# olsonanl/close_kmers

Measured on AMD Instinct MI355X. Metric: protein residues/s vs 1B-entry kmer image; 1/2/4/8 MI355X, higher is better.
Workload: dtype u64

## Files before the change

### close_kmers_amd/csrc/kgx_host_batch.cpp

```cpp
#include <hip/hip_runtime.h>

#include <algorithm>
#include <chrono>
#include <cstdio>
#include <cstdlib>
#include <cstring>
#include <string>
#include <vector>

#include "kgx_rt.h"

using namespace kgx;

extern "C" {


namespace {

void cut_at_nul(char *b, uint64_t len)
{
    const void *z = len ? std::memchr(b, 0, len) : nullptr;
    if (z) {
        const uint64_t slen = (uint64_t)((const char *)z - b);
        for (uint64_t i = slen ? slen - 1 : 0; i < len; i++)
// ... 870 lines not shown
    return KGX_OK;
}

hipError_t own_queue_stream(int device, hipStream_t *s)
{
    (void)device;
    const char *e = std::getenv("KGX_OWN_QUEUES");
    if (!e || std::atoi(e) != 0) {
        int least = 0, greatest = 0;
        if (hipDeviceGetStreamPriorityRange(&least, &greatest) == hipSuccess && least != greatest &&
            hipStreamCreateWithPriority(s, hipStreamNonBlocking, least) == hipSuccess)
            return hipSuccess;
        (void)hipGetLastError();
    }
    return hipStreamCreateWithFlags(s, hipStreamNonBlocking);
}

int process_batch_chunked(kgx_ctx *c, const kgx_params *params, const char *residues,
                          const uint64_t *seq_offsets, uint32_t n_seq, uint32_t want, uint32_t K,
                          kgx_result *out)
{
    if (!c->twin) {
        int rc = kgx_ctx_create(c->img, &c->twin);
        if (rc)
            return rc;
    }
    kgx_ctx *t = c->twin;
    t->opt.probe_variant = c->opt.probe_variant;
    t->opt.probe_j = c->opt.probe_j;
    t->opt.probe_filter = c->opt.probe_filter;
    t->opt.probe_serialize = c->opt.probe_serialize;
    t->opt.score_variant = c->opt.score_variant;
    t->opt.score_wave_tiles = c->opt.score_wave_tiles;
    kgx_ctx *xs[2] = {c, t};
    if (!c->copy_stream)
        HIP_TRY(own_queue_stream(c->img->device, &c->copy_stream));
    if (c->opt.host_upload_stream && !c->up_stream)
        HIP_TRY(own_queue_stream(c->img->device, &c->up_stream));
    for (auto *ev : {&c->chunk_counts, &c->chunk_gathered, &c->chunk_done, &c->chunk_h2d})
        if (int erc = ensure_events(*ev, K))
            return erc;

    const uint64_t r0 = seq_offsets[0], n_res = seq_offsets[n_seq] - r0;
    std::vector<uint32_t> cut(K + 1, 0);
    cut[K] = n_seq;
    const bool taper = c->opt.host_taper && K >= 3;
    const double wsum = taper ? (double)K - 1.0 : (double)K;
    for (uint32_t k = 1; k < K; k++) {
        const double before = taper ? 0.5 + (double)(k - 1) : (double)k;
        const uint64_t target = r0 + (uint64_t)((double)n_res * before / wsum);
        uint32_t s = (uint32_t)(std::lower_bound(seq_offsets, seq_offsets + n_seq + 1, target) - seq_offsets);
        cut[k] = std::min(std::max(s, cut[k - 1]), n_seq);
    }
    cut.erase(std::unique(cut.begin(), cut.end()), cut.end());
    K = (uint32_t)cut.size() - 1;
    const bool want_calls = (want & KGX_WANT_CALLS) != 0;
    const bool want_otu = (want & KGX_WANT_OTU) != 0;
    const bool need_hits = (want & KGX_WANT_HITS) != 0;
    const bool want_best = (want & KGX_WANT_BEST) != 0;
    uint64_t hbase = 0, cbase = 0, obase = 0, nwin = 0;
    const bool compact = c->opt.host_hits16 && need_hits && c->img->layout == KGX_LAYOUT_PACKED16;
    uint64_t mbase = 0;
    int rc = reset_chunked_results(c, n_seq, want_best, compact);
    if (rc)
        return rc;
    struct PoolDrain {
// ... 652 lines not shown
```

### close_kmers_amd/csrc/kgx_internal.h

```cpp
#ifndef KGX_INTERNAL_H
#define KGX_INTERNAL_H

#include <hip/hip_runtime.h>
#include <stdint.h>

#include "kgx.h"
#include "kgx_line_home.h"

namespace kgx {

constexpr int KMER = 8;
constexpr uint64_t CORE = 1280000000ULL;
constexpr uint64_t MAX_ENCODED = 25600000000ULL;
constexpr uint64_t EMPTY_KEY = MAX_ENCODED + 1;
constexpr int RUN_CAP = 40000 - 2;

constexpr int PROBE_WAVES = 4;
constexpr uint32_t HIT_PLANES = KGX_HIT_PLANES, HIT_PACKED16 = KGX_HIT_PACKED16;
constexpr int PROBE_BUCKET = 0;
constexpr int PROBE_KEY_FIRST = 1;
constexpr int PROBE_AUTO = -1;
constexpr int PROBE_LINE = 2;
constexpr int PROBE_LINE8 = 3;
constexpr int PROBE_J_DEFAULT = 2;
// ... 94 lines not shown
    uint32_t n_seq;
    uint64_t max_tiles;
};
struct ProbeHits {
    uint4 *hot, *cold;
    uint64_t *hit_mask;
};
struct ProbeRun {
    int probe_j;
    int variant;
    uint32_t lds_kb;
    uint32_t max_blocks;
    bool defer;
    uint32_t nt;
};
hipError_t launch_probe(const ProbeBatch &b, const ProbeTable &t, const ProbeHits &h, const ProbeRun &r,
                        hipStream_t stream);
hipError_t launch_probe_dna(const ProbeBatch &b, const ProbeTable &t, const ProbeHits &h, const ProbeRun &r,
                            hipStream_t stream);

hipError_t launch_pack(const kgx_sig_kmer *table, packed_bucket *packed, uint64_t n,
                       uint32_t *not_packable, hipStream_t stream);
hipError_t launch_unpack(const packed_bucket *packed, kgx_sig_kmer *out, uint64_t n,
                         hipStream_t stream);
hipError_t launch_filter_build(const void *table, int layout, uint64_t num_sigs, uint64_t *filter,
                               uint32_t log2_words, hipStream_t stream);

enum { SCORE_HYBRID = 0, SCORE_WAVE = 1, SCORE_LANE = 2, SCORE_WAVE_ONLY = 3  };
constexpr uint32_t LONG_SEQ = 2048;
hipError_t launch_score(uint32_t n_seq, uint64_t n_residues, const uint64_t *wbase, const uint32_t *tile_seq,
                        uint64_t max_tiles, const uint64_t *hit_mask, uint32_t tile_windows, uint4 *hot,
                        kgx_call *calls, void *ranges, uint32_t *hit_count, uint32_t *call_count,
                        kgx_params params, uint32_t want, uint32_t hit_format, int variant, uint32_t wave_tiles,
                        const uint32_t *plan_status, hipStream_t stream);
hipError_t launch_best_calls(uint32_t n_seq, const kgx_call *calls, const uint64_t *start, const uint32_t *count,
                             kgx_call *ws, kgx_best_call *out, hipStream_t stream);
hipError_t launch_otus(uint32_t n_seq, const uint64_t *wbase, const uint64_t *hit_mask, uint32_t tile_windows,
                       const uint4 *hot, const uint4 *cold, int32_t *ws, kgx_otu *otus, uint32_t *otu_count,
                       uint32_t hit_format, hipStream_t stream);

constexpr uint32_t SMALL_GATHER_SEQ = 256;
constexpr uint32_t SMALL_COLLECT_BEST_SEQ = 8192;
constexpr uint32_t SMALL_GATHER_BLOCKS = 64;
hipError_t launch_small_gather(uint32_t n, const uint64_t *wbase, const uint64_t *hit_mask, uint32_t tile_windows,
                               const uint32_t *hit_count, const uint32_t *call_count, const uint4 *hot,
                               const uint4 *cold, const kgx_call *calls, const uint32_t *otu_count,
                               const kgx_otu *otus, kgx_hit *hits_out, kgx_call *calls_out, kgx_otu *otus_out,
                               uint64_t *h0, uint64_t *h1, uint64_t *h2, const uint32_t *status,
                               const kgx_best_call *best, kgx_best_call *best_host, uint32_t *status_host,
                               uint64_t *nwin_host, uint32_t *done_host, uint32_t token, uint32_t *blocks_done,
                               uint32_t hit_format, hipStream_t stream);
hipError_t launch_gather(uint32_t n_seq, const uint64_t *wbase, const uint64_t *hit_mask,
                         uint32_t tile_windows, const uint32_t *call_count, const uint4 *hot, const uint4 *cold,
                         const kgx_call *calls, const uint64_t *hit_dense_off,
                         const uint64_t *call_dense_off, kgx_hit *hits_out, kgx_call *calls_out,
                         uint32_t seq_base, uint32_t hit_format, const uint32_t *otu_count, const kgx_otu *otus,
                         const uint64_t *otu_dense_off, kgx_otu *otus_out, hipStream_t stream,
                         uint4 *hits16_out = nullptr,
                         uint32_t *hits12_out = nullptr);
size_t count_scan_workspace_bytes(uint32_t n);
hipError_t launch_count_scan(uint32_t n, const uint32_t *c0, const uint32_t *c1, const uint32_t *c2, uint64_t *o0,
                             uint64_t *o1, uint64_t *o2, void *workspace, hipStream_t stream);
constexpr int SMALL_PIECES = 5;
struct SmallPieces {
    uint4 *dst[SMALL_PIECES];
    const uint4 *src[SMALL_PIECES];
    uint64_t end16[SMALL_PIECES];
// ... 99 lines not shown
```

### close_kmers_amd/csrc/kgx_options.h

```cpp
#pragma once

#include <cstdint>
#include <cstring>
#include <string>

namespace kgx {

inline bool probe_j_supported(int j) { return (j >= 1 && j <= 5) || j == 8; }

struct CtxOptions {
    int64_t probe_variant = -1;
    int64_t probe_j = 2;
    int64_t probe_lds_kb = 0;
    int64_t probe_persist = 0;
    int64_t probe_filter = 1;
    int64_t line_index = 1;
    int64_t probe_nt = 0;
    int64_t probe_serialize = 1;
    int64_t probe_stream = 0;
    int64_t plan_fused = 0;
    int64_t score_variant = 0;
    int64_t score_wave_tiles = 16;
    int64_t fq_residues = 1;
    int64_t fq_count = 1;
    int64_t fq_probe_j = 1;
    int64_t fq_plan = 1;
    int64_t fq_fused = 1;
    int64_t microbench_span = 0;
    int64_t microbench_ilp = 8;
    int64_t microbench_wgs = 8;
    int64_t host_chunks = 6;
    int64_t host_copy = 1;
    int64_t host_copy_blocks = 64;
    int64_t host_hits16 = 1;
    int64_t host_threads = 12;
    int64_t stage_threads = 8;
    int64_t host_upload_stream = 0;
    int64_t host_score_variant = 1;
    int64_t host_stream = 1;
    int64_t host_taper = 1;
    int64_t pinned_input = 1;
    int64_t host_rec12 = 1;
    int64_t host_h2d_first = 1;
    int64_t host_stage_all = 0;
    int64_t host_stream_dma = 0;
    int64_t host_nt = 1;
    int64_t counts_first = 1;
    int64_t host_profile = 0;
    int64_t small_batch = 1 << 21;
    int64_t small_wave = 1;
    int64_t small_wave_tiles = 1;
    int64_t small_fused = 0;
    int64_t fused_inline = 1;
    int64_t gunzip_device = 0;
};
// ... 26 lines not shown
    {KGX_OPT(stage_threads), 1, 64, "1..64", nullptr},
    {KGX_OPT(host_score_variant), -1, 2, "-1 (the context's score_variant) or 0..2", nullptr},
    {KGX_OPT(host_upload_stream), 0, 1, "0 or 1", nullptr},
    {KGX_OPT(host_stream_dma), 0, 1, "0 or 1", nullptr},
    {KGX_OPT(pinned_input), 0, 1, "0 or 1", nullptr},
    {KGX_OPT(host_stage_all), 0, 1, "0 or 1", nullptr},
    {KGX_OPT(host_h2d_first), 0, 1, "0 or 1", nullptr},
    {KGX_OPT(host_rec12), 0, 1, "0 or 1", nullptr},
    {KGX_OPT(host_nt), 0, 1, "0 or 1", nullptr},
    {KGX_OPT(host_taper), 0, 1, "0 or 1", nullptr},
    {KGX_OPT(host_stream), 0, 1, "0 or 1", nullptr},
    {KGX_OPT(counts_first), 0, 1, "0 or 1", nullptr},
    {KGX_OPT(host_threads), 1, 64, "1..64", nullptr},
    {KGX_OPT(small_batch), 0, 1 << 24, "0..16777216 residues", nullptr},
    {KGX_OPT(probe_stream), 0, 1, "0 or 1", nullptr},
    {KGX_OPT(probe_persist), 0, 32, "0..32 workgroups per CU", nullptr},
    {KGX_OPT(small_wave), 0, 1, "0 or 1", nullptr},
    {KGX_OPT(host_profile), 0, 1, "0 or 1", nullptr},
    {KGX_OPT(host_chunks), 1, 64, "1..64", nullptr},
    {KGX_OPT(fq_count), 0, 1, "0 or 1", nullptr},
    {KGX_OPT(fq_residues), 0, 1, "0 or 1", nullptr},
    {KGX_OPT(score_variant), 0, 2, "0, 1 or 2", nullptr},
    {KGX_OPT(probe_lds_kb), 0, 160, "0..160", nullptr},
    {KGX_OPT(fused_inline), 0, 1, "0 or 1", nullptr},
    {KGX_OPT(small_fused), 0, 1, "0 or 1", nullptr},
    {KGX_OPT(small_wave_tiles), 1, 256, "1..256", nullptr},
    {KGX_OPT(score_wave_tiles), 1, 256, "1..256", nullptr},
    {KGX_OPT(fq_fused), 0, 1, "0 or 1", nullptr},
    {KGX_OPT(fq_plan), 0, 1, "0 or 1", nullptr},
    {KGX_OPT(fq_probe_j), 0, 4, "0 (= probe_j), 1, 2, 3 or 4", nullptr},
    {KGX_OPT(probe_j), 0, 0, "1, 2, 3, 4, 5 or 8", probe_j_ok},
};
constexpr size_t CTX_OPTION_COUNT = sizeof(CTX_OPTION_TABLE) / sizeof(CTX_OPTION_TABLE[0]);
static const CtxOptionRow CTX_OPTION_TABLE_IO[] = {
    {KGX_OPT(gunzip_device), 0, 1, "0 or 1", nullptr},
};
#undef KGX_OPT

inline const CtxOptionRow *ctx_option_find(const char *name)
{
    for (const CtxOptionRow &r : CTX_OPTION_TABLE)
        if (!std::strcmp(r.name, name))
            return &r;
    for (const CtxOptionRow &r : CTX_OPTION_TABLE_IO)
        if (!std::strcmp(r.name, name))
            return &r;
    return nullptr;
}

inline int ctx_option_set(CtxOptions &o, const char *name, int64_t value, std::string *err)
{
    const CtxOptionRow *r = ctx_option_find(name);
    if (!r) {
        *err = std::string("unknown option ") + name;
        return -1;
    }
    if (r->ok ? !r->ok(value) : (value < r->lo || value > r->hi)) {
        *err = std::string(name) + " must be " + r->must_be;
        return -1;
    }
    o.*(r->field) = value;
    return 0;
}

inline bool ctx_option_get(const CtxOptions &o, const char *name, int64_t *value)
{
    const CtxOptionRow *r = ctx_option_find(name);
    if (r)
        *value = o.*(r->field);
    return r != nullptr;
}

}
```

### close_kmers_amd/csrc/kgx_rt.h

```cpp
#ifndef KGX_RT_H
#define KGX_RT_H

#include <hip/hip_runtime.h>

#include <algorithm>
#include <atomic>
#include <chrono>
#include <condition_variable>
#include <cstdio>
#include <cstdlib>
#include <cstring>
#include <deque>
#include <functional>
#include <memory>
#include <mutex>
#include <string>
#include <thread>
#include <vector>

#include "kgx_internal.h"
#include "kgx_options.h"

namespace kgx {

// ... 373 lines not shown
        fqc_calls;
    kgx::PinnedVec<uint32_t> h_fqc_n, h_fqc_reads, h_fqc_fc, h_fqc_len;
    kgx::PinnedVec<uint64_t> h_fqc_tot, h_fqc_fo, h_fqc_coff;
    kgx::PinnedVec<kgx_call> h_fqc_calls;
    kgx::CtxOptions opt;
    bool probe_defer = true;
    std::vector<uint64_t> h_hoff, h_coff, h_ooff;
    kgx::PinnedVec<kgx_hit> h_hits;
    kgx::PinnedVec<kgx_call> h_calls;
    kgx::PinnedVec<kgx_otu> h_otus;
    kgx::PinnedVec<uint32_t> h_ocount;
    kgx::DevBuf otu_ws, otus, otu_count, dense_ooff, dense_otus;
    bool have_otus = false;
    kgx::PinnedVec<uint32_t> h_hcount, h_ccount;
    kgx::PinnedVec<char> h_res;
    kgx_ctx *twin = nullptr;
    kgx::PinnedVec<uint64_t> h_off_stage, h_dense_hoff, h_dense_coff, h_dense_ooff, h_nwin;
    std::unique_ptr<kgx::HostPool> pool;
    std::unique_ptr<kgx::HostPool> stage_pool;
    kgx::PinnedVec<uint4> h_hits16;
    kgx::PinnedVec<uint64_t> h_mask;
    std::vector<uint64_t> h_wstart;
    std::vector<hipEvent_t> chunk_done;
    std::vector<hipEvent_t> chunk_counts;
    std::vector<hipEvent_t> chunk_gathered;
    hipStream_t copy_stream = nullptr;
    hipStream_t up_stream = nullptr;
    kgx::DevBuf up_res, up_off;
    kgx::DevBuf dense_mask, dense_best;
    double rate_hits = 0.35, rate_calls = 0.05, rate_otus = 0.05;
    uint64_t stream_fallbacks = 0;
    bool one_pass_pinned = false;
    uint64_t pinned_batches = 0, nul_reruns = 0;
    uint32_t counts_enqueued = 0;
    kgx::PinnedVec<uint32_t> h_nul;
    std::vector<hipEvent_t> chunk_h2d;
    kgx::DevBuf dense_counts, cscan_ws;
    kgx::PinnedVec<uint32_t> h_counts;
    kgx::PinnedVec<uint32_t> h_hits12;
    kgx::PinnedVec<char> h_res_all;
    kgx::PinnedVec<uint64_t> h_off_all;
    kgx::PinnedVec<uint4> h_small;
    kgx::PinnedVec<uint32_t> h_done;
    kgx::DevBuf small_blocks_done;
    uint64_t fused_batches = 0, small_batches = 0;
    kgx::PinnedVec<uint64_t> h_fwb;
    kgx::PinnedVec<kgx_hit> h_fhits;
    kgx::PinnedVec<kgx_call> h_fcalls;
    kgx::PinnedVec<uint32_t> h_fcounts, h_fdone;
    kgx::PinnedVec<uint64_t> h_fdbg;
    uint32_t small_token = 0;
    kgx::PinnedVec<kgx_call> h_calls_region;
    kgx::PinnedVec<kgx_otu> h_otus_region;
    int compact_out = 0;
    struct CompactSeg {
        uint32_t s0, s1, words;
        uint64_t hit_begin, rec_at, mask_at;
    };
    std::vector<CompactSeg> compact_segs;
    std::vector<kgx_hit_chunk> compact_chunks;
    std::vector<hipEvent_t> prof_ev;
    std::vector<hipEvent_t> prof_done;
    kgx_host_profile last_profile{};
    std::unique_ptr<kgx::RollupScratch> rollup;
};

// ... 55 lines not shown
```

### close_kmers_amd/csrc/kgx_runtime.cpp

```cpp
#include <hip/hip_runtime.h>
#include <sched.h>

#include <algorithm>
#include <cerrno>
#include <ctime>
#include <chrono>
#include <cstdio>
#include <cstdlib>
#include <cstring>
#include <map>
#include <stdexcept>
#include <string>
#include <atomic>
#include <fcntl.h>
#include <mutex>
#include <sys/stat.h>
#include <thread>
#include <unistd.h>
#include <vector>

#include "kgx_rt.h"

using namespace kgx;

// ... 831 lines not shown
    bool ok = std::fwrite(&h, sizeof(h), 1, f) == 1;
    const uint64_t chunk = 1ull << 25;
    std::vector<kgx_sig_kmer> buf(std::min(chunk, std::max<uint64_t>(img->num_sigs, 1)));
    for (uint64_t b = 0; ok && b < img->num_sigs; b += chunk) {
        const uint64_t m = std::min(chunk, img->num_sigs - b);
        int rc = image_read(img, b, m, buf.data());
        if (rc) {
            std::fclose(f);
            return rc;
        }
        ok = std::fwrite(buf.data(), sizeof(kgx_sig_kmer), m, f) == m;
    }
    if (std::fclose(f) != 0)
        ok = false;
    return ok ? KGX_OK : fail(KGX_EIO, "short write to " + path);
}


int kgx_ctx_create(kgx_image *img, kgx_ctx **out)
{
    if (!img || !out)
        return fail(KGX_EINVAL, "null argument");
    HIP_TRY(hipSetDevice(img->device));
    bool probe_defer = true;
    if (int rc = env_switch("KGX_PROBE_DEFER", "rounds per slice", "deferred", probe_defer))
        return rc;
    int64_t gunzip_device = CtxOptions{}.gunzip_device;
    if (const char *g = std::getenv("KGX_GUNZIP_DEVICE")) {
        if (*g && std::strcmp(g, "0") && std::strcmp(g, "1"))
            return fail(KGX_EINVAL, std::string("KGX_GUNZIP_DEVICE: 0 (host threads) or 1 (device), not \"") + g + "\"");
        if (*g)
            gunzip_device = *g == '1';
    }
    kgx_ctx *c = new kgx_ctx;
    c->img = img;
    c->probe_defer = probe_defer;
    c->opt.gunzip_device = gunzip_device;
    hipError_t e = hipStreamCreateWithFlags(&c->stream, hipStreamNonBlocking);
    if (e != hipSuccess) {
        delete c;
        return fail(KGX_EDEVICE, std::string("stream: ") + hipGetErrorString(e));
    }
    c->own_stream = true;
    if (const char *sb = std::getenv("KGX_SMALL_BATCH"))
        c->opt.small_batch = std::min<int64_t>(1 << 24, std::max<int64_t>(0, std::atoll(sb)));
    e = hipEventCreateWithFlags(&c->probe_done, hipEventDisableTiming);
    if (e != hipSuccess) {
        (void)hipStreamDestroy(c->stream);
        delete c;
        return fail(KGX_EDEVICE, std::string("event: ") + hipGetErrorString(e));
    }
    *out = c;
    return KGX_OK;
}

int kgx_ctx_destroy(kgx_ctx *c)
{
    if (!c)
        return KGX_OK;
    (void)hipSetDevice(c->img->device);
    if (c->twin)
        kgx_ctx_destroy(c->twin);
    (void)hipStreamSynchronize(c->stream);
    for (DevBuf *b : {&c->residues, &c->offsets, &c->wbase, &c->tile_seq, &c->hit_mask,
                      &c->hits, &c->calls, &c->hit_count, &c->call_count, &c->dense_hoff,
                      &c->dense_coff, &c->dense_hits, &c->dense_calls, &c->plan_ws, &c->ranges})
        b->release();
    {
        std::lock_guard<std::mutex> lock(c->img->probe_mu);
        if (c->img->last_probe == c->probe_done)
// ... 246 lines not shown
    return probe_chained(c, [&] {
        const CtxProbe p = ctx_probe(c, bases, n_bases, anchors);
        return launch_probe_dna(p.batch, ctx_probe_table(c), p.hits, p.run, c->stream);
    });
}

}

extern "C" {

int kgx_stage_probe(kgx_ctx *c, const uint8_t *d_res, const uint64_t *d_off)
{
    if (!c || (!d_res && c->n_residues) || d_off != c->d_off)
        return fail(KGX_EINVAL, "probe: residues missing or offsets differ from the plan");
    return probe_chained(c, [&] {
        const CtxProbe p = ctx_probe(c, d_res, c->n_residues, d_off);
        return launch_probe(p.batch, ctx_probe_table(c), p.hits, p.run, c->stream);
    });
}



int kgx_stage_score(kgx_ctx *c, const kgx_params *params, uint32_t want)
{
    if (!c)
        return fail(KGX_EINVAL, "null ctx");
    kgx_params p;
    if (params)
        p = *params;
    else
        kgx_params_default(&p);
    HIP_TRY(hipSetDevice(c->img->device));
    const bool best = (want & KGX_WANT_BEST) != 0;
    HIP_TRY(launch_score(c->n_seq, c->n_residues, c->wbase.as<uint64_t>(), c->tile_seq.as<uint32_t>(), c->max_tiles,
                         c->hit_mask.as<uint64_t>(), c->tile_windows, c->hits.as<uint4>(), c->calls.as<kgx_call>(),
                         c->ranges.p, c->hit_count.as<uint32_t>(), c->call_count.as<uint32_t>(), p,
                         want | (best ? KGX_WANT_CALLS : 0u), c->hit_format, c->opt.score_variant,
                         (uint32_t)c->opt.score_wave_tiles, c->plan_status.as<uint32_t>(), c->stream));
    c->have_best = false;
    c->have_otus = false;
    if (want & KGX_WANT_OTU) {
        HIP_TRY(c->otu_ws.reserve(std::max<uint64_t>(c->hit_slots, 1) * sizeof(int32_t)));
        HIP_TRY(c->otus.reserve(std::max<uint64_t>(c->hit_slots, 1) * sizeof(kgx_otu)));
        HIP_TRY(c->otu_count.reserve(std::max<uint64_t>(c->n_seq, 1) * sizeof(uint32_t)));
        HIP_TRY(launch_otus(c->n_seq, c->wbase.as<uint64_t>(), c->hit_mask.as<uint64_t>(), c->tile_windows,
                            c->hits.as<uint4>(), c->hits.as<uint4>() + c->hit_slots, c->otu_ws.as<int32_t>(),
                            c->otus.as<kgx_otu>(), c->otu_count.as<uint32_t>(), c->hit_format, c->stream));
        c->have_otus = true;
    }
    if (best) {
        HIP_TRY(c->best.reserve(std::max<uint64_t>(c->n_seq, 1) * sizeof(kgx_best_call)));
        HIP_TRY(c->best_ws.reserve(c->hit_slots * sizeof(kgx_call)));
        if (!c->defer_best)
            HIP_TRY(launch_best_calls(c->n_seq, c->calls.as<kgx_call>(), c->wbase.as<uint64_t>(),
                                      c->call_count.as<uint32_t>(), c->best_ws.as<kgx_call>(),
                                      c->best.as<kgx_best_call>(), c->stream));
        c->have_best = true;
    }
    return KGX_OK;
}

int kgx_find_best_calls(kgx_ctx *c, const kgx_call *calls, const uint64_t *call_offsets, uint32_t n_seq,
                        kgx_best_call *out)
{
    if (!c || (n_seq && (!call_offsets || !out)))
        return fail(KGX_EINVAL, "null argument");
    if (n_seq == 0)
        return KGX_OK;
    const uint64_t c0 = call_offsets[0], n = call_offsets[n_seq] - c0;
    if (n && !calls)
        return fail(KGX_EINVAL, "null calls");
// ... 90 lines not shown
                               c->tile_windows, c->plan_status.as<uint32_t>(), c->plan_ws.as<uint32_t>(), c->stream);
        if (e != hipSuccess)
            rc = fail(KGX_EDEVICE, std::string("fq plan: ") + hipGetErrorString(e));
    }
    if (!rc)
        rc = stage_probe_dna(c, fr->bases, fr->n_bases, fr->anchors, fr->offsets);
    c->opt.probe_j = keep_j;
    if (rc)
        return rc;
    if ((rc = kgx_stage_score(c, params, want)))
        return rc;
    return out ? kgx_device_result_get(c, out) : KGX_OK;
}

}

extern "C" {

int kgx_ctx_stat(kgx_ctx *c, const char *name, int64_t *value)
{
    if (!c || !name || !value)
        return fail(KGX_EINVAL, "null argument");
    const std::string n = name;
    if (n == "fused_batches")
        *value = (int64_t)c->fused_batches;
    else if (n == "small_batches")
        *value = (int64_t)c->small_batches;
    else if (n == "stream_fallbacks")
        *value = (int64_t)c->stream_fallbacks;
    else if (n == "pinned_batches")
        *value = (int64_t)c->pinned_batches;
    else if (n == "nul_reruns")
        *value = (int64_t)c->nul_reruns;
    else
        return fail(KGX_EINVAL, "unknown statistic " + n);
    return KGX_OK;
}

int kgx_ctx_host_profile(kgx_ctx *c, kgx_host_profile *out)
{
    if (!c || !out)
        return fail(KGX_EINVAL, "null argument");
    *out = c->last_profile;
    return KGX_OK;
}

int kgx_device_batch_collect(kgx_ctx *c, uint32_t want, kgx_result *out)
{
    if (!c || !out)
        return fail(KGX_EINVAL, "null argument");
    if (!c->have_hits)
        return fail(KGX_EINVAL, "no device batch to collect");
    const bool want_calls = (want & KGX_WANT_CALLS) != 0;
    const bool want_otu = (want & KGX_WANT_OTU) != 0;
    const bool need_hits = (want & KGX_WANT_HITS) != 0;
    const bool want_best = (want & KGX_WANT_BEST) != 0;
    if (want_otu && !c->have_otus)
        return fail(KGX_EINVAL, "no device OTU tallies (score with KGX_WANT_OTU)");
    if (want_best && !c->have_best)
        return fail(KGX_EINVAL, "no device best calls (score with KGX_WANT_BEST)");
    HIP_TRY(hipSetDevice(c->img->device));
    PhaseTimer tm(c);
    const uint32_t n_seq = c->n_seq;
    const bool best_now = want_best && n_seq && !need_hits && !want_calls && !want_otu;
    if (c->counts_enqueued != want + 1) {
        if (int rc = kgx::collect_counts_enqueue(c, want))
// ... 233 lines not shown
```

### close_kmers_amd/csrc/kgx_score.hip

```cpp
#include "kgx_device.h"
#include "kgx_lstd.h"

namespace kgx {


template <class F>
__device__ __forceinline__ uint32_t for_each_run(const uint64_t *__restrict__ hit_mask,
                                                 uint32_t tile_windows, uint64_t gw0, uint64_t gw1,
                                                 F &&f)
{
    if (gw0 >= gw1)
        return 0;
    const uint32_t J = tile_windows / 64;
    const uint64_t gfirst = gw0 >> 6, glast = (gw1 - 1) >> 6;
    uint64_t tile = gfirst / J;
    uint32_t pre = 0;
    for (uint64_t g = tile * J; g < gfirst; g++)
        pre += (uint32_t)__popcll(hit_mask[g]);
    uint32_t ordinal = 0;
    uint64_t next = hit_mask[gfirst];
    for (uint64_t g = gfirst; g <= glast; g++) {
        if (g != gfirst && g % J == 0) {
            tile = g / J;
            pre = 0;
        }
        const uint64_t full = next;
        if (g < glast)
            next = hit_mask[g + 1];
        const uint32_t lo = g == gfirst ? (uint32_t)(gw0 & 63) : 0u;
        const uint32_t hi = g == glast ? (uint32_t)((gw1 - 1) & 63) + 1 : 64u;
        const uint64_t bits = full & bit_range(lo, hi);
        const uint32_t cnt = (uint32_t)__popcll(bits);
        if (cnt)
            f(tile * tile_windows + pre + (uint32_t)__popcll(full & bit_range(0, lo)), cnt, ordinal, bits,
              (uint32_t)(64 * g - gw0));
        ordinal += cnt;
        pre += (uint32_t)__popcll(full);
    }
    return ordinal;
}


struct RunTail {
    uint32_t pos, fI, idx;
    float wt;
    uint32_t avg;
    uint32_t fb;
    uint64_t at;
};

constexpr int SCORE_BATCH = 8;

template <bool PK, int SB = SCORE_BATCH>
__device__ __forceinline__ void score_sequence(
    uint32_t s, const uint64_t *__restrict__ wbase, const uint64_t *__restrict__ hit_mask,
    uint32_t tile_windows, uint4 *__restrict__ hot, kgx_call *__restrict__ calls,
    uint2 *__restrict__ ranges, uint32_t *__restrict__ hit_count, uint32_t *__restrict__ call_count,
    const kgx_params &prm, uint32_t want)
{
    const uint64_t gw0 = wbase[s], gw1 = wbase[s + 1];
    const bool want_calls = (want & KGX_WANT_CALLS) != 0;
    const bool want_otu = (want & KGX_WANT_OTU) != 0;
    if (!want_calls && !want_otu) {
        hit_count[s] = for_each_run(hit_mask, tile_windows, gw0, gw1,
                                    [](uint64_t, uint32_t, uint32_t, uint64_t, uint32_t) {});
        call_count[s] = 0;
        return;
    }
    if (!want_otu && prm.min_hits > 0 && gw1 > gw0) {
        uint32_t nh = 0;
        for (uint64_t g = gw0 >> 6; g <= (gw1 - 1) >> 6; g++) {
            const uint32_t lo = g == (gw0 >> 6) ? (uint32_t)(gw0 & 63) : 0u;
            const uint32_t hi = g == ((gw1 - 1) >> 6) ? (uint32_t)((gw1 - 1) & 63) + 1 : 64u;
            nh += (uint32_t)__popcll(hit_mask[g] & bit_range(lo, hi));
        }
        if ((int)nh < prm.min_hits) {
            hit_count[s] = nh;
            call_count[s] = 0;
            return;
        }
    }

    typedef HitFields<PK> HF;
    constexpr uint32_t F_RUN = KGX_HIT_IN_RUN << HF::FLAG_SHIFT, F_CNT = KGX_HIT_COUNTED << HF::FLAG_SHIFT,
                       F_OTU = KGX_HIT_OTU << HF::FLAG_SHIFT;
    constexpr int FD = HF::FLAG_DWORD;
    uint32_t *hw = reinterpret_cast<uint32_t *>(hot);
    const uint64_t cbase = gw0;
    const uint32_t gap = (uint32_t)prm.max_gap;
    int n = 0;
    uint32_t cur = 0, first_pos = 0, last_pos = 0, last_idx = 0, run_start = 0;
    int cnt = 0;
    float wsum = 0.0f;
    RunTail p1 = {0, 0, 0, 0.0f, 0, 0, 0}, p2 = {0, 0, 0, 0.0f, 0, 0, 0};
    uint32_t ncalls = 0;

    auto flush = [&]() {
        if (n == 0)
            return;
        if (cnt >= prm.min_hits && wsum >= (float)prm.min_weighted_hits) {
            if (want_calls) {
                kgx_call cl;
                cl.start = first_pos;
                cl.end = last_pos + (KMER - 1);
                cl.count = cnt;
                cl.function_index = cur;
                cl.weighted_hits = wsum;
                calls[cbase + ncalls] = cl;
            }
            if (want_otu)
                ranges[cbase + ncalls] = make_uint2(run_start, last_idx);
            ncalls++;
        }
        if (n >= 2 && p2.fI != cur && p2.fI == p1.fI) {
            cur = p1.fI;
            n = 2;
            run_start = p2.idx;
            first_pos = p2.pos;
            cnt = 2;
            wsum = 0.0f + p2.wt;
            wsum = wsum + p1.wt;
            last_pos = p1.pos;
            last_idx = p1.idx;
            if (want_otu) {
                hw[4 * p2.at + FD] = p2.fb | F_RUN | F_CNT;
                hw[4 * p1.at + FD] = p1.fb | F_RUN | F_CNT;
            }
        } else {
            n = 0;
        }
    };

    auto step = [&](const uint4 &r, uint32_t i, uint64_t at, uint32_t pos) {
        const uint32_t avg = HF::avg(r);
        const uint32_t fI = HF::fi(r);
        const float wt = __uint_as_float(HF::wt(r));
        const uint32_t fb = HF::flag_base(r);
        if (n > 0 && p1.pos + gap < pos) {
            if (n >= prm.min_hits)
                flush();
            else
                n = 0;
        }
        if (n == 0) {
            cur = fI;
            cnt = 0;
            wsum = 0.0f;
            run_start = i;
            first_pos = pos;
        }
        bool accept = true;
        if (prm.order_constraint && n > 0) {
            const uint32_t d = (pos - p1.pos) - (uint32_t)((int)p1.avg - (int)avg);
            accept = (fI == p1.fI) && d <= 20u;
        }
        if (accept) {
            if (n < RUN_CAP) {
                n++;
                const bool counted = fI == cur;
                if (want_otu)
                    hw[4 * at + FD] = fb | F_RUN | (counted ? F_CNT : 0u);
                if (counted) {
                    cnt++;
                    wsum += wt;
                    last_pos = pos;
                    last_idx = i;
                }
                p2 = p1;
                p1 = RunTail{pos, fI, i, wt, avg, fb, at};
            }
            if (n > 1 && cur != fI && p2.fI == p1.fI)
                flush();
        }
    };

    auto load_batch = [&](uint4 *rb, uint64_t at0, uint32_t b, uint32_t c) {
#pragma unroll
        for (int k = 0; k < SB; k++)
            if (b + k < c)
                rb[k] = hot[at0 + b + k];
    };
    const uint32_t nh = for_each_run(hit_mask, tile_windows, gw0, gw1,
                                     [&](uint64_t at0, uint32_t c, uint32_t ord0, uint64_t bits, uint32_t pbase) {
        uint4 ra[SB], rb[SB];
        load_batch(ra, at0, 0, c);
        for (uint32_t b = 0; b < c; b += 2 * SB) {
            if (b + SB < c)
                load_batch(rb, at0, b + SB, c);
#pragma unroll
            for (int k = 0; k < SB; k++)
                if (b + k < c) {
                    step(ra[k], ord0 + b + k, at0 + b + k, pbase + (uint32_t)__builtin_ctzll(bits));
                    bits &= bits - 1;
                }
            if (b + SB >= c)
                break;
            if (b + 2 * SB < c)
                load_batch(ra, at0, b + 2 * SB, c);
#pragma unroll
            for (int k = 0; k < SB; k++)
                if (b + SB + k < c) {
                    step(rb[k], ord0 + b + SB + k, at0 + b + SB + k,
                         pbase + (uint32_t)__builtin_ctzll(bits));
                    bits &= bits - 1;
                }
        }
    });
    if (n >= prm.min_hits)
        flush();
    hit_count[s] = nh;
    call_count[s] = want_calls ? ncalls : 0;

    if (want_otu && ncalls > 0) {
        uint32_t ci = 0;
        uint2 rg = ranges[cbase];
        const uint32_t end = ranges[cbase + ncalls - 1].y;
        for_each_run(hit_mask, tile_windows, gw0, gw1,
                     [&](uint64_t at0, uint32_t c, uint32_t ord0, uint64_t, uint32_t) {
            for (uint32_t k = 0; k < c; k++) {
                const uint32_t i = ord0 + k;
                if (i > end)
                    return;
                while (i > rg.y)
                    rg = ranges[cbase + ++ci];
                if (i >= rg.x) {
                    const uint32_t f = hw[4 * (at0 + k) + FD];
                    if (f & F_CNT)
                        hw[4 * (at0 + k) + FD] = f | F_OTU;
                }
            }
        });
    }
}

template <bool PK, int SB>
__global__ __launch_bounds__(256) void score_kernel(
    uint32_t n_seq, const uint64_t *__restrict__ wbase, const uint64_t *__restrict__ hit_mask,
    uint32_t tile_windows, uint4 *__restrict__ hot, kgx_call *__restrict__ calls,
    uint2 *__restrict__ ranges, uint32_t *__restrict__ hit_count, uint32_t *__restrict__ call_count,
    kgx_params prm, uint32_t want, uint32_t skip_above)
{
    for (uint32_t s = blockIdx.x * blockDim.x + threadIdx.x; s < n_seq; s += gridDim.x * blockDim.x) {
        const uint64_t w = wbase[s + 1] - wbase[s];
        if (w > skip_above && w <= (uint64_t)RUN_CAP)
            continue;
        score_sequence<PK, SB>(s, wbase, hit_mask, tile_windows, hot, calls, ranges, hit_count, call_count, prm,
                               want);
    }
}


constexpr uint32_t SQ = 256;

struct ScoreQueue {
    uint32_t pos[SQ];
    uint32_t seq[SQ];
    uint32_t at[SQ];
    uint64_t mw[64];
    uint64_t wb[65];
};


__device__ __forceinline__ uint32_t seq_lower_bound(const uint64_t *__restrict__ wbase,
                                                    const uint32_t *__restrict__ tile_seq, uint32_t T, uint64_t x)
{
    uint32_t s = tile_seq[x / T];
    if (wbase[s] < x)
        return s + 1;
    while (s > 0 && wbase[s - 1] == x)
        s--;
    return s;
}

template <bool PK>
__global__ __launch_bounds__(256) void score_wave_kernel(
    uint32_t n_seq, const uint64_t *__restrict__ wbase, const uint32_t *__restrict__ tile_seq,
    const uint64_t *__restrict__ hit_mask, uint32_t tile_windows, uint32_t wave_tiles, uint4 *__restrict__ hot,
    kgx_call *__restrict__ calls, uint32_t *__restrict__ hit_count, uint32_t *__restrict__ call_count,
    kgx_params prm, uint32_t want, uint32_t only_above, const uint32_t *__restrict__ plan_status)
{
// ... 299 lines not shown
    }
    flush_counts(s_hi);
    if (!scoring)
        return;
    if (qtail != qissue)
        issue(qtail - qissue);
    if (npend) {
        wave_lds_sync();
        process_chunk(npend, rpend);
    }
    if (o_valid) {
        close_open();
        if (lane == 0)
            call_count[o_seq] = want_calls ? o_ncalls : 0u;
    }
}

template <bool PK>
__global__ __launch_bounds__(256) void score_long_kernel(
    uint32_t n_seq, const uint64_t *__restrict__ wbase, const uint64_t *__restrict__ hit_mask,
    uint32_t tile_windows, uint4 *__restrict__ hot, kgx_call *__restrict__ calls,
    uint2 *__restrict__ ranges, uint32_t *__restrict__ hit_count, uint32_t *__restrict__ call_count,
    kgx_params prm, uint32_t want)
{
    const uint32_t s = blockIdx.x * blockDim.x + threadIdx.x;
    if (s < n_seq && wbase[s + 1] - wbase[s] > (uint64_t)RUN_CAP)
        score_sequence<PK>(s, wbase, hit_mask, tile_windows, hot, calls, ranges, hit_count, call_count, prm, want);
}

hipError_t launch_score(uint32_t n_seq, uint64_t n_residues, const uint64_t *wbase, const uint32_t *tile_seq,
                        uint64_t max_tiles, const uint64_t *hit_mask, uint32_t tile_windows, uint4 *hot,
                        kgx_call *calls, void *ranges, uint32_t *hit_count, uint32_t *call_count,
                        kgx_params params, uint32_t want, uint32_t hit_format, int variant, uint32_t wave_tiles,
                        const uint32_t *plan_status, hipStream_t stream)
{
    if (n_seq == 0)
        return hipSuccess;
    const bool pk = hit_format == HIT_PACKED16;
    const dim3 lanes((n_seq + 255) / 256);
    const bool wave_ok = !params.order_constraint && max_tiles * tile_windows < (1ull << 32);
    wave_tiles = std::max<uint32_t>(1, wave_tiles);
    const uint64_t waves = std::max<uint64_t>(1, (max_tiles + wave_tiles - 1) / wave_tiles);
    const dim3 wgrid((uint32_t)((waves + 3) / 4));
#define KGX_WAVE(P, ABOVE)                                                                                      \
    hipLaunchKernelGGL(score_wave_kernel<P>, wgrid, dim3(256), 0, stream, n_seq, wbase, tile_seq, hit_mask,     \
                       tile_windows, wave_tiles, hot, calls, hit_count, call_count, params, want, (ABOVE), plan_status)
    if (variant == SCORE_WAVE_ONLY && wave_ok) {
        if (pk)
            KGX_WAVE(true, 0u);
        else
            KGX_WAVE(false, 0u);
        return hipGetLastError();
    }
    if ((variant == SCORE_WAVE || variant == SCORE_WAVE_ONLY) && wave_ok) {
        if (pk) {
            KGX_WAVE(true, 0u);
            hipLaunchKernelGGL(score_long_kernel<true>, lanes, dim3(256), 0, stream, n_seq, wbase, hit_mask,
                               tile_windows, hot, calls, static_cast<uint2 *>(ranges), hit_count, call_count, params,
                               want);
        } else {
            KGX_WAVE(false, 0u);
            hipLaunchKernelGGL(score_long_kernel<false>, lanes, dim3(256), 0, stream, n_seq, wbase, hit_mask,
                               tile_windows, hot, calls, static_cast<uint2 *>(ranges), hit_count, call_count, params,
                               want);
        }
        return hipGetLastError();
    }
    const bool hybrid = variant == SCORE_HYBRID && wave_ok;
    const uint32_t skip = hybrid ? LONG_SEQ : ~0u;
    const bool small = n_residues < 64ull * n_seq;
    static const uint32_t grid_cap = [] {
        const char *e = std::getenv("KGX_SCORE_GRID_CAP");
        return e ? (uint32_t)std::max(0L, std::strtol(e, nullptr, 10)) : 0u;
    }();
    const dim3 sgrid(grid_cap ? std::min<uint32_t>(lanes.x, grid_cap) : lanes.x);
#define KGX_SCORE(P, B)                                                                                          \
    hipLaunchKernelGGL((score_kernel<P, B>), sgrid, dim3(256), 0, stream, n_seq, wbase, hit_mask, tile_windows, hot, \
                       calls, static_cast<uint2 *>(ranges), hit_count, call_count, params, want, skip)
    if (pk && small)
        KGX_SCORE(true, 2);
    else if (pk)
        KGX_SCORE(true, SCORE_BATCH);
    else if (small)
        KGX_SCORE(false, 2);
    else
        KGX_SCORE(false, SCORE_BATCH);
#undef KGX_SCORE
    if (hybrid) {
        if (pk)
            KGX_WAVE(true, LONG_SEQ);
        else
            KGX_WAVE(false, LONG_SEQ);
    }
#undef KGX_WAVE
    return hipGetLastError();
}

__global__ __launch_bounds__(256) void best_call_kernel(uint32_t n_seq, const kgx_call *__restrict__ calls,
                                                        const uint64_t *__restrict__ start,
                                                        const uint32_t *__restrict__ count, kgx_call *__restrict__ ws,
                                                        kgx_best_call *__restrict__ out)
{
    const uint32_t s = blockIdx.x * blockDim.x + threadIdx.x;
    if (s < n_seq)
        out[s] = best_call_decide(calls + start[s], count[s], ws + start[s]);
}

hipError_t launch_best_calls(uint32_t n_seq, const kgx_call *calls, const uint64_t *start, const uint32_t *count,
                             kgx_call *ws, kgx_best_call *out, hipStream_t stream)
{
    if (n_seq == 0)
        return hipSuccess;
    hipLaunchKernelGGL(best_call_kernel, dim3((n_seq + 255) / 256), dim3(256), 0, stream, n_seq, calls, start,
                       count, ws, out);
    return hipGetLastError();
}


constexpr int64_t OTU_LDS = 24;
// ... 80 lines not shown
```

Before: 64.74 billion.

## Add lean lane scorer with 32-bit indices, narrow hit loads, optional wave compaction

Result: faster. 66.79 billion, median of 6 (+3.2%).

```diff
diff --git a/close_kmers_amd/csrc/kgx_host_batch.cpp b/close_kmers_amd/csrc/kgx_host_batch.cpp
--- a/close_kmers_amd/csrc/kgx_host_batch.cpp
+++ b/close_kmers_amd/csrc/kgx_host_batch.cpp
@@ -926,6 +926,7 @@
     t->opt.probe_serialize = c->opt.probe_serialize;
     t->opt.score_variant = c->opt.score_variant;
     t->opt.score_wave_tiles = c->opt.score_wave_tiles;
+    t->opt.score_lean = c->opt.score_lean;
     kgx_ctx *xs[2] = {c, t};
     if (!c->copy_stream)
         HIP_TRY(own_queue_stream(c->img->device, &c->copy_stream));
diff --git a/close_kmers_amd/csrc/kgx_internal.h b/close_kmers_amd/csrc/kgx_internal.h
--- a/close_kmers_amd/csrc/kgx_internal.h
+++ b/close_kmers_amd/csrc/kgx_internal.h
@@ -150,7 +150,7 @@
                         uint64_t max_tiles, const uint64_t *hit_mask, uint32_t tile_windows, uint4 *hot,
                         kgx_call *calls, void *ranges, uint32_t *hit_count, uint32_t *call_count,
                         kgx_params params, uint32_t want, uint32_t hit_format, int variant, uint32_t wave_tiles,
-                        const uint32_t *plan_status, hipStream_t stream);
+                        int lean, const uint32_t *plan_status, hipStream_t stream, bool *lean_taken = nullptr);
 hipError_t launch_best_calls(uint32_t n_seq, const kgx_call *calls, const uint64_t *start, const uint32_t *count,
                              kgx_call *ws, kgx_best_call *out, hipStream_t stream);
 hipError_t launch_otus(uint32_t n_seq, const uint64_t *wbase, const uint64_t *hit_mask, uint32_t tile_windows,
diff --git a/close_kmers_amd/csrc/kgx_options.h b/close_kmers_amd/csrc/kgx_options.h
--- a/close_kmers_amd/csrc/kgx_options.h
+++ b/close_kmers_amd/csrc/kgx_options.h
@@ -21,6 +21,7 @@
     int64_t plan_fused = 0;
     int64_t score_variant = 0;
     int64_t score_wave_tiles = 16;
+    int64_t score_lean = 1;
     int64_t fq_residues = 1;
     int64_t fq_count = 1;
     int64_t fq_probe_j = 1;
@@ -113,8 +114,9 @@
     {KGX_OPT(probe_j), 0, 0, "1, 2, 3, 4, 5 or 8", probe_j_ok},
 };
 constexpr size_t CTX_OPTION_COUNT = sizeof(CTX_OPTION_TABLE) / sizeof(CTX_OPTION_TABLE[0]);
-static const CtxOptionRow CTX_OPTION_TABLE_IO[] = {
+static const CtxOptionRow CTX_OPTION_TABLE_LATER[] = {
     {KGX_OPT(gunzip_device), 0, 1, "0 or 1", nullptr},
+    {KGX_OPT(score_lean), 0, 2, "0, 1 or 2", nullptr},
 };
 #undef KGX_OPT
 
@@ -123,7 +125,7 @@
     for (const CtxOptionRow &r : CTX_OPTION_TABLE)
         if (!std::strcmp(r.name, name))
             return &r;
-    for (const CtxOptionRow &r : CTX_OPTION_TABLE_IO)
+    for (const CtxOptionRow &r : CTX_OPTION_TABLE_LATER)
         if (!std::strcmp(r.name, name))
             return &r;
     return nullptr;
diff --git a/close_kmers_amd/csrc/kgx_rt.h b/close_kmers_amd/csrc/kgx_rt.h
--- a/close_kmers_amd/csrc/kgx_rt.h
+++ b/close_kmers_amd/csrc/kgx_rt.h
@@ -429,6 +429,7 @@
     uint64_t stream_fallbacks = 0;
     bool one_pass_pinned = false;
     uint64_t pinned_batches = 0, nul_reruns = 0;
+    uint64_t lean_scores = 0;
     uint32_t counts_enqueued = 0;
     kgx::PinnedVec<uint32_t> h_nul;
     std::vector<hipEvent_t> chunk_h2d;
diff --git a/close_kmers_amd/csrc/kgx_runtime.cpp b/close_kmers_amd/csrc/kgx_runtime.cpp
--- a/close_kmers_amd/csrc/kgx_runtime.cpp
+++ b/close_kmers_amd/csrc/kgx_runtime.cpp
@@ -887,10 +887,19 @@
         if (*g)
             gunzip_device = *g == '1';
     }
+    int64_t score_lean = CtxOptions{}.score_lean;
+    if (const char *l = std::getenv("KGX_SCORE_LEAN")) {
+        if (*l && std::strcmp(l, "0") && std::strcmp(l, "1") && std::strcmp(l, "2"))
+            return fail(KGX_EINVAL, std::string("KGX_SCORE_LEAN: 0 (general lane scorer), 1 (lean) or 2 (lean, "
+                                                "packed), not \"") + l + "\"");
+        if (*l)
+            score_lean = *l - '0';
+    }
     kgx_ctx *c = new kgx_ctx;
     c->img = img;
     c->probe_defer = probe_defer;
     c->opt.gunzip_device = gunzip_device;
+    c->opt.score_lean = score_lean;
     hipError_t e = hipStreamCreateWithFlags(&c->stream, hipStreamNonBlocking);
     if (e != hipSuccess) {
         delete c;
@@ -1203,11 +1212,14 @@
         kgx_params_default(&p);
     HIP_TRY(hipSetDevice(c->img->device));
     const bool best = (want & KGX_WANT_BEST) != 0;
+    bool lean_taken = false;
     HIP_TRY(launch_score(c->n_seq, c->n_residues, c->wbase.as<uint64_t>(), c->tile_seq.as<uint32_t>(), c->max_tiles,
                          c->hit_mask.as<uint64_t>(), c->tile_windows, c->hits.as<uint4>(), c->calls.as<kgx_call>(),
                          c->ranges.p, c->hit_count.as<uint32_t>(), c->call_count.as<uint32_t>(), p,
                          want | (best ? KGX_WANT_CALLS : 0u), c->hit_format, c->opt.score_variant,
-                         (uint32_t)c->opt.score_wave_tiles, c->plan_status.as<uint32_t>(), c->stream));
+                         (uint32_t)c->opt.score_wave_tiles, (int)c->opt.score_lean, c->plan_status.as<uint32_t>(),
+                         c->stream, &lean_taken));
+    c->lean_scores += lean_taken;
     c->have_best = false;
     c->have_otus = false;
     if (want & KGX_WANT_OTU) {
@@ -1364,6 +1376,8 @@
         *value = (int64_t)c->pinned_batches;
     else if (n == "nul_reruns")
         *value = (int64_t)c->nul_reruns;
+    else if (n == "lean_scores")
+        *value = (int64_t)c->lean_scores;
     else
         return fail(KGX_EINVAL, "unknown statistic " + n);
     return KGX_OK;
diff --git a/close_kmers_amd/csrc/kgx_score.hip b/close_kmers_amd/csrc/kgx_score.hip
--- a/close_kmers_amd/csrc/kgx_score.hip
+++ b/close_kmers_amd/csrc/kgx_score.hip
@@ -1,5 +1,7 @@
 #include "kgx_device.h"
 #include "kgx_lstd.h"
+
+#include <type_traits>
 
 namespace kgx {
 
@@ -40,6 +42,35 @@
     return ordinal;
 }
 
+template <class F>
+__device__ __forceinline__ uint32_t for_each_run_lean(const uint64_t *__restrict__ hit_mask,
+                                                      uint32_t tile_windows, uint32_t gw0, uint32_t gw1,
+                                                      F &&f)
+{
+    if (gw0 >= gw1)
+        return 0;
+    const uint32_t J = tile_windows / 64;
+    const uint32_t gfirst = gw0 >> 6, glast = (gw1 - 1) >> 6;
+    uint32_t slot = gfirst / J * tile_windows;
+    for (uint32_t g = gfirst / J * J; g < gfirst; g++)
+        slot += (uint32_t)__popcll(hit_mask[g]);
+    uint32_t ordinal = 0;
+    for (uint32_t g = gfirst; g <= glast; g++) {
+        if (g != gfirst && g % J == 0)
+            slot = g / J * tile_windows;
+        const uint64_t full = hit_mask[g];
+        const uint32_t lo = g == gfirst ? (gw0 & 63) : 0u;
+        const uint32_t hi = g == glast ? ((gw1 - 1) & 63) + 1 : 64u;
+        const uint64_t bits = full & bit_range(lo, hi);
+        const uint32_t cnt = (uint32_t)__popcll(bits);
+        if (cnt)
+            f(slot + (uint32_t)__popcll(full & bit_range(0, lo)), cnt, ordinal, bits, 64 * g - gw0);
+        ordinal += cnt;
+        slot += (uint32_t)__popcll(full);
+    }
+    return ordinal;
+}
+
 
 struct RunTail {
     uint32_t pos, fI, idx;
@@ -50,43 +81,66 @@
 };
 
 constexpr int SCORE_BATCH = 8;
-
-template <bool PK, int SB = SCORE_BATCH>
-__device__ __forceinline__ void score_sequence(
+constexpr int SCORE_LEAN_BATCH = 4;
+
+struct __attribute__((packed, aligned(4))) HitYZ {
+    uint32_t y, z;
+};
+__device__ __forceinline__ uint2 load_yz(const uint4 *rec)
+{
+    const HitYZ v = *reinterpret_cast<const HitYZ *>(reinterpret_cast<const uint32_t *>(rec) + 1);
+    return make_uint2(v.y, v.z);
+}
+__device__ __forceinline__ const uint4 &as_hit(const uint4 &r) { return r; }
+__device__ __forceinline__ uint4 as_hit(const uint2 &r) { return make_uint4(0u, r.x, r.y, 0u); }
+
+template <bool PK, int SB = SCORE_BATCH, bool LEAN = false, bool EARLY = true, bool RUNS = true>
+__device__ __forceinline__ bool score_sequence(
     uint32_t s, const uint64_t *__restrict__ wbase, const uint64_t *__restrict__ hit_mask,
     uint32_t tile_windows, uint4 *__restrict__ hot, kgx_call *__restrict__ calls,
     uint2 *__restrict__ ranges, uint32_t *__restrict__ hit_count, uint32_t *__restrict__ call_count,
     const kgx_params &prm, uint32_t want)
 {
-    const uint64_t gw0 = wbase[s], gw1 = wbase[s + 1];
-    const bool want_calls = (want & KGX_WANT_CALLS) != 0;
-    const bool want_otu = (want & KGX_WANT_OTU) != 0;
-    if (!want_calls && !want_otu) {
-        hit_count[s] = for_each_run(hit_mask, tile_windows, gw0, gw1,
-                                    [](uint64_t, uint32_t, uint32_t, uint64_t, uint32_t) {});
-        call_count[s] = 0;
-        return;
-    }
-    if (!want_otu && prm.min_hits > 0 && gw1 > gw0) {
-        uint32_t nh = 0;
-        for (uint64_t g = gw0 >> 6; g <= (gw1 - 1) >> 6; g++) {
-            const uint32_t lo = g == (gw0 >> 6) ? (uint32_t)(gw0 & 63) : 0u;
-            const uint32_t hi = g == ((gw1 - 1) >> 6) ? (uint32_t)((gw1 - 1) & 63) + 1 : 64u;
-            nh += (uint32_t)__popcll(hit_mask[g] & bit_range(lo, hi));
-        }
-        if ((int)nh < prm.min_hits) {
-            hit_count[s] = nh;
+    typedef typename std::conditional<LEAN, uint32_t, uint64_t>::type Idx;
+    const Idx gw0 = (Idx)wbase[s], gw1 = (Idx)wbase[s + 1];
+    auto each_run = [&](auto &&f) {
+        if constexpr (LEAN)
+            return for_each_run_lean(hit_mask, tile_windows, gw0, gw1, f);
+        else
+            return for_each_run(hit_mask, tile_windows, gw0, gw1, f);
+    };
+    const bool want_calls = LEAN || (want & KGX_WANT_CALLS) != 0;
+    const bool want_otu = !LEAN && (want & KGX_WANT_OTU) != 0;
+    if (EARLY) {
+        if (!want_calls && !want_otu) {
+            hit_count[s] = each_run([](Idx, uint32_t, uint32_t, uint64_t, uint32_t) {});
             call_count[s] = 0;
-            return;
-        }
-    }
+            return false;
+        }
+        if (!want_otu && prm.min_hits > 0 && gw1 > gw0) {
+            uint32_t nh = 0;
+            for (Idx g = gw0 >> 6; g <= (gw1 - 1) >> 6; g++) {
+                const uint32_t lo = g == (gw0 >> 6) ? (uint32_t)(gw0 & 63) : 0u;
+                const uint32_t hi = g == ((gw1 - 1) >> 6) ? (uint32_t)((gw1 - 1) & 63) + 1 : 64u;
+                nh += (uint32_t)__popcll(hit_mask[g] & bit_range(lo, hi));
+            }
+            if ((int)nh < prm.min_hits) {
+                hit_count[s] = nh;
+                call_count[s] = 0;
+                return false;
+            }
+        }
+    }
+    if (!RUNS)
+        return true;
+    typedef typename std::conditional<LEAN, uint2, uint4>::type Rec;
 
     typedef HitFields<PK> HF;
     constexpr uint32_t F_RUN = KGX_HIT_IN_RUN << HF::FLAG_SHIFT, F_CNT = KGX_HIT_COUNTED << HF::FLAG_SHIFT,
                        F_OTU = KGX_HIT_OTU << HF::FLAG_SHIFT;
     constexpr int FD = HF::FLAG_DWORD;
     uint32_t *hw = reinterpret_cast<uint32_t *>(hot);
-    const uint64_t cbase = gw0;
+    const Idx cbase = gw0;
     const uint32_t gap = (uint32_t)prm.max_gap;
     int n = 0;
     uint32_t cur = 0, first_pos = 0, last_pos = 0, last_idx = 0, run_start = 0;
@@ -131,7 +185,8 @@
         }
     };
 
-    auto step = [&](const uint4 &r, uint32_t i, uint64_t at, uint32_t pos) {
+    auto step = [&](const Rec &rec, uint32_t i, Idx at, uint32_t pos) {
+        const auto &r = as_hit(rec);
         const uint32_t avg = HF::avg(r);
         const uint32_t fI = HF::fi(r);
         const float wt = __uint_as_float(HF::wt(r));
@@ -150,7 +205,7 @@
             first_pos = pos;
         }
         bool accept = true;
-        if (prm.order_constraint && n > 0) {
+        if (!LEAN && prm.order_constraint && n > 0) {
             const uint32_t d = (pos - p1.pos) - (uint32_t)((int)p1.avg - (int)avg);
             accept = (fI == p1.fI) && d <= 20u;
         }
@@ -174,15 +229,19 @@
         }
     };
 
-    auto load_batch = [&](uint4 *rb, uint64_t at0, uint32_t b, uint32_t c) {
+    auto load_batch = [&](Rec *rb, Idx at0, uint32_t b, uint32_t c) {
 #pragma unroll
         for (int k = 0; k < SB; k++)
-            if (b + k < c)
-                rb[k] = hot[at0 + b + k];
+            if (b + k < c) {
+                if constexpr (LEAN)
+                    rb[k] = load_yz(hot + (at0 + b + k));
+                else
+                    rb[k] = hot[at0 + b + k];
+            }
     };
-    const uint32_t nh = for_each_run(hit_mask, tile_windows, gw0, gw1,
-                                     [&](uint64_t at0, uint32_t c, uint32_t ord0, uint64_t bits, uint32_t pbase) {
-        uint4 ra[SB], rb[SB];
+    const uint32_t nh = each_run(
+                                     [&](Idx at0, uint32_t c, uint32_t ord0, uint64_t bits, uint32_t pbase) {
+        Rec ra[SB], rb[SB];
         load_batch(ra, at0, 0, c);
         for (uint32_t b = 0; b < c; b += 2 * SB) {
             if (b + SB < c)
@@ -216,7 +275,7 @@
         uint2 rg = ranges[cbase];
         const uint32_t end = ranges[cbase + ncalls - 1].y;
         for_each_run(hit_mask, tile_windows, gw0, gw1,
-                     [&](uint64_t at0, uint32_t c, uint32_t ord0, uint64_t, uint32_t) {
+                     [&](Idx at0, uint32_t c, uint32_t ord0, uint64_t, uint32_t) {
             for (uint32_t k = 0; k < c; k++) {
                 const uint32_t i = ord0 + k;
                 if (i > end)
@@ -231,6 +290,7 @@
             }
         });
     }
+    return true;
 }
 
 template <bool PK, int SB>
@@ -246,6 +306,48 @@
             continue;
         score_sequence<PK, SB>(s, wbase, hit_mask, tile_windows, hot, calls, ranges, hit_count, call_count, prm,
                                want);
+    }
+}
+
+template <bool PK, int SB, bool PACK>
+__global__ __launch_bounds__(256) __attribute__((amdgpu_waves_per_eu(8, 8))) void score_lean_kernel(
+    uint32_t n_seq, const uint64_t *__restrict__ wbase, const uint64_t *__restrict__ hit_mask,
+    uint32_t tile_windows, uint4 *__restrict__ hot, kgx_call *__restrict__ calls,
+    uint32_t *__restrict__ hit_count, uint32_t *__restrict__ call_count, kgx_params prm, uint32_t want,
+    uint32_t skip_above)
+{
+    __shared__ uint32_t stay_seq[4][64];
+    __shared__ uint32_t stay_n[4];
+    for (uint64_t base = (uint64_t)blockIdx.x * 256u; base < n_seq; base += (uint64_t)gridDim.x * 256u) {
+        uint32_t s = (uint32_t)min(base + threadIdx.x, (uint64_t)n_seq);
+        bool stay = false;
+        if (s < n_seq) {
+            const uint64_t w = wbase[s + 1] - wbase[s];
+            stay = !(w > skip_above && w <= (uint64_t)RUN_CAP) &&
+                   score_sequence<PK, SB, true, true, false>(s, wbase, hit_mask, tile_windows, hot, calls, nullptr,
+                                                             hit_count, call_count, prm, want);
+        }
+        if constexpr (PACK) {
+            const uint32_t wave = threadIdx.x >> 6;
+            const uint64_t m = __ballot(stay);
+            if (stay)
+                stay_seq[wave][lanes_below(m)] = s;
+            if (lane_id() == 0)
+                stay_n[wave] = (uint32_t)__popcll(m);
+            __syncthreads();
+            uint32_t i = threadIdx.x, w = 0;
+            while (w < 4 && i >= stay_n[w])
+                i -= stay_n[w++];
+            stay = w < 4;
+            if (stay)
+                s = stay_seq[w][i];
+        }
+        if (stay)
+            score_sequence<PK, SB, true, false, true>(s, wbase, hit_mask, tile_windows, hot, calls, nullptr, hit_count,
+                                                call_count, prm, want);
+        if constexpr (PACK)
+            if (base + (uint64_t)gridDim.x * 256u < n_seq)
+                __syncthreads();
     }
 }
 
@@ -611,8 +713,10 @@
                         uint64_t max_tiles, const uint64_t *hit_mask, uint32_t tile_windows, uint4 *hot,
                         kgx_call *calls, void *ranges, uint32_t *hit_count, uint32_t *call_count,
                         kgx_params params, uint32_t want, uint32_t hit_format, int variant, uint32_t wave_tiles,
-                        const uint32_t *plan_status, hipStream_t stream)
-{
+                        int lean, const uint32_t *plan_status, hipStream_t stream, bool *lean_taken)
+{
+    if (lean_taken)
+        *lean_taken = false;
     if (n_seq == 0)
         return hipSuccess;
     const bool pk = hit_format == HIT_PACKED16;
@@ -656,14 +760,32 @@
 #define KGX_SCORE(P, B)                                                                                          \
     hipLaunchKernelGGL((score_kernel<P, B>), sgrid, dim3(256), 0, stream, n_seq, wbase, hit_mask, tile_windows, hot, \
                        calls, static_cast<uint2 *>(ranges), hit_count, call_count, params, want, skip)
+#define KGX_LEAN(P, B, PACK)                                                                                     \
+    hipLaunchKernelGGL((score_lean_kernel<P, B, PACK>), sgrid, dim3(256), 0, stream, n_seq, wbase, hit_mask,     \
+                       tile_windows, hot, calls, hit_count, call_count, params, want, skip)
+#define KGX_LANES(P, B, LB)                                                                                       \
+    do {                                                                                                         \
+        if (lean_ok && lean >= 2)                                                                                \
+            KGX_LEAN(P, LB, true);                                                                               \
+        else if (lean_ok)                                                                                        \
+            KGX_LEAN(P, LB, false);                                                                              \
+        else                                                                                                     \
+            KGX_SCORE(P, B);                                                                                     \
+    } while (0)
+    const bool lean_ok = lean > 0 && (want & KGX_WANT_CALLS) && !(want & KGX_WANT_OTU) && params.order_constraint == 0 &&
+                         max_tiles * tile_windows < (1ull << 32);
+    if (lean_taken)
+        *lean_taken = lean_ok;
     if (pk && small)
-        KGX_SCORE(true, 2);
+        KGX_LANES(true, 2, 2);
     else if (pk)
-        KGX_SCORE(true, SCORE_BATCH);
+        KGX_LANES(true, SCORE_BATCH, SCORE_LEAN_BATCH);
     else if (small)
-        KGX_SCORE(false, 2);
+        KGX_LANES(false, 2, 2);
     else
-        KGX_SCORE(false, SCORE_BATCH);
+        KGX_LANES(false, SCORE_BATCH, SCORE_LEAN_BATCH);
+#undef KGX_LANES
+#undef KGX_LEAN
 #undef KGX_SCORE
     if (hybrid) {
         if (pk)
```
